# himhan34/Intensity_based_LiDAR_SLAM_for_me-

Measured on NVIDIA B200. Metric: scan-to-map registrations/sec (OS0-64 frame, 100k-pt map), higher is better.
Workload: dtype f32 k-NN / f64 fit+solve

## Files before the change

### include/ilsm.h

```cpp
#ifndef ILSM_H_
#define ILSM_H_

#include <stddef.h>
#include <stdint.h>

#ifdef __cplusplus
extern "C" {
#endif

#define ILSM_ABI_VERSION 1

#if defined(__GNUC__)
#define ILSM_API __attribute__((visibility("default")))
#else
#define ILSM_API
#endif

typedef enum ilsm_status {
  ILSM_OK = 0,
  ILSM_ERR_INVALID_ARG = -1,
  ILSM_ERR_CUDA = -2,
  ILSM_ERR_NO_DEVICE = -3,
  ILSM_ERR_NOT_ENOUGH_MAP = -4,
  ILSM_ERR_OUT_OF_MEMORY = -5,
// ... 6 lines not shown
  ILSM_FAILURE = 2
} ilsm_termination;

typedef struct ilsm_ctx ilsm_ctx;
typedef struct ilsm_map ilsm_map;

ILSM_API int ilsm_abi_version(void);
ILSM_API const char* ilsm_last_error(void);

ILSM_API int ilsm_create(int device, ilsm_ctx** out);
ILSM_API void ilsm_destroy(ilsm_ctx* ctx);
ILSM_API int ilsm_sync(ilsm_ctx* ctx);
ILSM_API int ilsm_set_async(ilsm_ctx* ctx, int on);
ILSM_API void* ilsm_stream(ilsm_ctx* ctx);

ILSM_API int ilsm_host_register(void* ptr, size_t bytes);
ILSM_API int ilsm_host_unregister(void* ptr);

ILSM_API int ilsm_map_create(ilsm_ctx* ctx, ilsm_map** out);
ILSM_API void ilsm_map_destroy(ilsm_map* map);
ILSM_API int ilsm_map_size(const ilsm_map* map);

ILSM_API int ilsm_map_build(ilsm_map* map, const float* xyz, int n, int stride_bytes, float cell);
ILSM_API int ilsm_map_build_dev(ilsm_map* map, const float* d_xyz, int n, int stride_bytes, float cell);
ILSM_API int ilsm_map_build_pair_dev(ilsm_map* map_a, const float* d_xyz_a, int n_a, ilsm_map* map_b, const float* d_xyz_b, int n_b,
                                     int stride_bytes, float cell);
ILSM_API int ilsm_map_join(ilsm_map* map);

#define ILSM_INSERT_APPEND 0
#define ILSM_INSERT_NEAREST_TO_CENTRE 1
ILSM_API int ilsm_map_insert(ilsm_map* map, const float* xyz, int n, int stride_bytes, int policy, float leaf);

ILSM_API int ilsm_map_points(ilsm_map* map, float* out_xyzi, int capacity, int* n_out);

ILSM_API int ilsm_knn(ilsm_map* map, const float* q_xyz, int nq, int stride_bytes, int k, float max_dist, int32_t* idx,
             float* d2);
ILSM_API int ilsm_knn_dev(ilsm_map* map, const float* d_q_xyz, int nq, int stride_bytes, int k, float max_dist,
                 int32_t* d_idx, float* d_d2);

typedef struct ilsm_reg_opts {
  int32_t outer_iterations;
  int32_t max_num_iterations;
  double huber_a;
  float knn_gate_sq;
  float reserved0;
  double line_eig_ratio;
  double plane_tol;
  int32_t min_corner_map;
  int32_t min_surf_map;
} ilsm_reg_opts;

ILSM_API void ilsm_reg_opts_default(ilsm_reg_opts* o);

typedef struct ilsm_solve_summary {
  int32_t termination;
  int32_t iterations;
  int32_t num_successful_steps;
  int32_t num_unsuccessful_steps;
  int32_t num_edge_factors;
  int32_t num_plane_factors;
  int32_t num_evaluations;
  int32_t reserved;
  double initial_cost;
  double final_cost;
} ilsm_solve_summary;

// ... 285 lines not shown
```

### intensity_based_lidar_slam_for_me-_b200/binding.py

```python
from __future__ import annotations

import ctypes as C
import os

import numpy as np

from . import _build

ILSM_OK = 0
ILSM_ERR_NOT_ENOUGH_MAP = -4
CONVERGENCE, NO_CONVERGENCE, FAILURE = 0, 1, 2
MAX_OUTER = 8


class IlsmError(RuntimeError):
    def __init__(self, code, msg):
        super().__init__(f"ilsm error {code}: {msg}")
        self.code = code


class RegOpts(C.Structure):
    _fields_ = [("outer_iterations", C.c_int32), ("max_num_iterations", C.c_int32), ("huber_a", C.c_double),
                ("knn_gate_sq", C.c_float), ("reserved0", C.c_float), ("line_eig_ratio", C.c_double),
                ("plane_tol", C.c_double), ("min_corner_map", C.c_int32), ("min_surf_map", C.c_int32)]
# ... 64 lines not shown

def pc2_layout_ouster() -> Pc2Layout:
    lay = Pc2Layout()
    load_library().ilsm_pc2_layout_ouster(C.byref(lay))
    return lay


def load_library(path: str | None = None):
    global _lib
    if _lib is not None:
        return _lib
    path = path or _build.LIB
    if not os.path.exists(path):
        raise IlsmError(-100, f"{path} not built; run `python -c 'import __graft_entry__ as g; g.build()'`")
    lib = C.CDLL(path)
    vp, i32, f32, f64 = C.c_void_p, C.c_int, C.c_float, C.c_double
    sig = {
        "ilsm_abi_version": (i32, []),
        "ilsm_last_error": (C.c_char_p, []),
        "ilsm_create": (i32, [i32, C.POINTER(vp)]),
        "ilsm_destroy": (None, [vp]),
        "ilsm_sync": (i32, [vp]),
        "ilsm_stream": (vp, [vp]),
        "ilsm_set_async": (i32, [vp, i32]),
        "ilsm_map_create": (i32, [vp, C.POINTER(vp)]),
        "ilsm_map_destroy": (None, [vp]),
        "ilsm_map_size": (i32, [vp]),
        "ilsm_map_build": (i32, [vp, vp, i32, i32, f32]),
        "ilsm_map_build_dev": (i32, [vp, vp, i32, i32, f32]),
        "ilsm_map_join": (i32, [vp]),
        "ilsm_knn": (i32, [vp, vp, i32, i32, i32, f32, vp, vp]),
        "ilsm_map_insert": (i32, [vp, vp, i32, i32, i32, f32]),
        "ilsm_map_points": (i32, [vp, vp, i32, C.POINTER(i32)]),
        "ilsm_knn_dev": (i32, [vp, vp, i32, i32, i32, f32, vp, vp]),
        "ilsm_reg_opts_default": (None, [C.POINTER(RegOpts)]),
        "ilsm_register": (i32, [vp, vp, vp, vp, i32, vp, i32, i32, vp, vp, C.POINTER(RegOpts), C.POINTER(RegReport)]),
        "ilsm_register_dev": (i32, [vp, vp, vp, vp, i32, vp, i32, i32, vp, C.POINTER(RegOpts), vp]),
        "ilsm_associate": (i32, [vp, vp, vp, vp, i32, vp, i32, i32, vp, vp, C.POINTER(RegOpts), vp, vp, vp]),
        "ilsm_project": (i32, [vp, vp, i32, i32, i32, vp, vp, vp]),
        "ilsm_project_dev": (i32, [vp, vp, i32, i32, i32, vp, vp, vp]),
        "ilsm_extract_features": (i32, [vp, vp, i32, i32, f32, C.POINTER(Features)]),
        "ilsm_voxelgrid": (i32, [vp, vp, i32, i32, f32, vp, C.POINTER(i32)]),
        "ilsm_map_build_pair_dev": (i32, [vp, vp, i32, vp, vp, i32, i32, C.c_float]),
        "ilsm_register_frame": (i32, [vp, vp, vp, vp, i32, i32, C.c_float, C.c_float, C.c_float, vp, vp, vp, vp, vp]),
        "ilsm_register_frame_dev": (i32, [vp, vp, vp, vp, i32, i32, C.c_float, C.c_float, C.c_float, vp, vp]),
        "ilsm_sc_create": (i32, [vp, C.POINTER(vp)]),
        "ilsm_sc_destroy": (None, [vp]),
        "ilsm_sc_size": (i32, [vp]),
        "ilsm_sc_make": (i32, [vp, vp, i32, i32, vp]),
        "ilsm_sc_add": (i32, [vp, vp, i32]),
        "ilsm_sc_add_dev": (i32, [vp, vp, i32]),
        "ilsm_sc_query_topk": (i32, [vp, vp, i32, i32, i32, vp, vp, vp]),
        "ilsm_sc_query_topk_dev": (i32, [vp, vp, i32, i32, i32, vp, vp, vp]),
        "ilsm_sc_merge_topk_dev": (i32, [vp, vp, i32, i32, vp]),
        "ilsm_sc_merge_topk": (i32, [vp, vp, vp, i32, i32, vp, vp, vp]),
        "ilsm_sc_query_candidates": (i32, [vp, vp, i32, i32, vp, vp, vp, vp]),
        "ilsm_sc_query_topk_batch": (i32, [vp, vp, i32, i32, i32, i32, vp, vp, vp]),
        "ilsm_sc_query_topk_batch_dev": (i32, [vp, vp, i32, i32, i32, i32, vp]),
        "ilsm_sc_prefilter_debug": (i32, [vp, vp, i32, i32, vp, vp]),
        "ilsm_sc_nccl_unique_id": (i32, [vp]),
        "ilsm_sc_init_nccl_rank": (i32, [vp, vp, i32, i32]),
        "ilsm_sc_init_nccl": (i32, [vp, vp, i32, i32]),
        "ilsm_sc_nccl_version": (i32, [vp]),
        "ilsm_sc_query_topk_sharded": (i32, [vp, vp, i32, i32, i32, i32, vp, vp, vp]),
        "ilsm_sc_query_topk_sharded_dev": (i32, [vp, vp, i32, i32, i32, i32, vp]),
        "ilsm_odometry": (i32, [vp, vp, vp, vp, i32, vp, i32, i32, vp, vp, C.POINTER(RegOpts), C.POINTER(RegReport), vp]),
# ... 300 lines not shown
        return int(self._lib.ilsm_map_size(self._h))

    def set_input_cloud(self, cloud, cell: float = 0.0):
        a, n, stride = _cloud(cloud)
        _check(self._lib.ilsm_map_build(self._h, _ptr(a), n, stride, cell))
        return self

    build = set_input_cloud

    def build_dev(self, d_ptr: int, n: int, stride: int, cell: float = 0.0):
        _check(self._lib.ilsm_map_build_dev(self._h, d_ptr, n, stride, cell))
        return self

    def build_pair_dev(self, d_ptr: int, n: int, other: "LocalMap", d_ptr_other: int, n_other: int, stride: int, cell: float = 0.0):
        _check(self._lib.ilsm_map_build_pair_dev(self._h, d_ptr, n, other._h, d_ptr_other, n_other, stride, cell))
        return self

    def join(self):
        _check(self._lib.ilsm_map_join(self._h))
        return self

    def add_points(self, cloud, downsample=True, downsample_size=0.4):
        a, n, stride = _cloud(cloud)
        _check(self._lib.ilsm_map_insert(self._h, _ptr(a), n, stride, 1 if downsample else 0, downsample_size))
        return self

    def points(self):
        n = C.c_int(0)
        _check(self._lib.ilsm_map_points(self._h, None, 0, C.byref(n)))
        out = np.empty((max(n.value, 1), 4), np.float32)
        _check(self._lib.ilsm_map_points(self._h, _ptr(out), n.value, C.byref(n)))
        return out[:n.value]

    def nearest_k_search(self, queries, k: int = 5, max_dist: float = 0.0):
        q, nq, stride = _cloud(queries)
        idx = np.empty((nq, k), np.int32)
        d2 = np.empty((nq, k), np.float32)
        _check(self._lib.ilsm_knn(self._h, _ptr(q), nq, stride, k, max_dist, _ptr(idx), _ptr(d2)))
        return idx, d2

    def knn_dev(self, d_q_ptr: int, nq: int, stride: int, k: int, max_dist: float, d_idx_ptr: int, d_d2_ptr: int):
        _check(self._lib.ilsm_knn_dev(self._h, d_q_ptr, nq, stride, k, max_dist, d_idx_ptr, d_d2_ptr))


def merge_topk(dist, ids, shifts, k):
    d = np.ascontiguousarray(dist, np.float64).ravel()
    i = np.ascontiguousarray(ids, np.int32).ravel()
    s = np.ascontiguousarray(shifts, np.int32).ravel()
    od, oi, os_ = np.zeros(k), np.zeros(k, np.int32), np.zeros(k, np.int32)
    _check(load_library().ilsm_sc_merge_topk(_ptr(d), _ptr(i), _ptr(s), len(d), k, _ptr(od), _ptr(oi), _ptr(os_)))
    return od, oi, os_


class ScanContextDb:
    NUM_EXCLUDE_RECENT = 50
    SC_DIST_THRES = 0.13

    def __init__(self, ctx: Context):
        self._ctx = ctx
        self._lib = ctx._lib
        h = C.c_void_p()
        _check(self._lib.ilsm_sc_create(ctx._h, C.byref(h)))
        self._h = h

    def close(self):
        if getattr(self, "_h", None) and getattr(self._ctx, "_h", None):
# ... 334 lines not shown
```

### intensity_based_lidar_slam_for_me-_b200/csrc/api.cu

```cuda
#include <stdio.h>
#include <string.h>

#include <atomic>
#include <new>

#include "ilsm_host.hpp"

namespace ilsm {

static thread_local char g_err[512] = "";

int fail(int code, const char* msg) {
  snprintf(g_err, sizeof(g_err), "%s", msg);
  return code;
}
int fail_cuda(cudaError_t e, const char* where) {
  snprintf(g_err, sizeof(g_err), "CUDA error %d (%s) at %s", (int)e, cudaGetErrorString(e), where);
  cudaGetLastError();
  return ILSM_ERR_CUDA;
}
static std::atomic<long long> g_launches{0};
void count_launches(int k) { g_launches.fetch_add(k, std::memory_order_relaxed); }

int check_launch(const char* where) {
  cudaError_t e = cudaGetLastError();
  if (e != cudaSuccess) return fail_cuda(e, where);
  return ILSM_OK;
}

int eval_only_launch(Ctx* c, double* d_out, const double* d_pose7 = nullptr, double huber_a = 0.0);
int factors_export(Ctx* c, ilsm_factor* d_out);
int sc_merge_dev(Ctx* ctx, const void* d_packed, int shards, int k, void* d_out, int batch = 1, size_t shard_stride = 0);
void sc_nccl_release(ScDb& d);

struct Pose7 {
  double v[7];
};
// ... 20 lines not shown
    else if (t < 7) pose7[t] = st->xt[t - 4];
    if (report) {
      const int words = (int)(sizeof(ilsm_reg_report) / 4);
      const int32_t* src = reinterpret_cast<const int32_t*>(&st->report);
      int32_t* dst = reinterpret_cast<int32_t*>(report);
      for (int w = t; w < words; w += blockDim.x) dst[w] = src[w];
    }
  }
}

int Ctx::init(int dev) {
  int count = 0;
  cudaError_t e = cudaGetDeviceCount(&count);
  if (e != cudaSuccess || count <= 0) {
    cudaGetLastError();
    return fail(ILSM_ERR_NO_DEVICE, "no CUDA device available (libilsm_cuda has no CPU fallback)");
  }
  if (dev < 0 || dev >= count) return fail(ILSM_ERR_INVALID_ARG, "ilsm_create: device index out of range");
  device = dev;
  ILSM_CUDA(cudaSetDevice(dev));
  cudaDeviceProp prop;
  ILSM_CUDA(cudaGetDeviceProperties(&prop, dev));
  sm_count = prop.multiProcessorCount;
  ILSM_CUDA(cudaStreamCreateWithFlags(&stream, cudaStreamNonBlocking));
  ILSM_CUDA(cudaStreamCreateWithFlags(&aux, cudaStreamNonBlocking));
  ILSM_CUDA(cudaEventCreateWithFlags(&ev_fork, cudaEventDisableTiming));
  ILSM_CUDA(cudaEventCreateWithFlags(&ev_join, cudaEventDisableTiming));
  int rc;
  if ((rc = lm.reserve(1))) return rc;
  ILSM_CUDA(cudaMemsetAsync(lm.p, 0, sizeof(LmState), stream));
  if ((rc = pinned.reserve(4096))) return rc;
  ILSM_CUDA(cudaStreamSynchronize(stream));
  if (const char* e2 = getenv("ILSM_KNN_BINNED_MIN")) knn_binned_min = atoi(e2) > 0 ? atoi(e2) : 0x7fffffff;
  if (const char* e3 = getenv("ILSM_KNN_GROUP")) {
    const int gsz = atoi(e3);
    if (gsz == 1 || gsz == 2 || gsz == 4 || gsz == 8 || gsz == 16 || gsz == 32) knn_group = gsz;
  }
  return ILSM_OK;
}

void Ctx::release() {
  if (fe_graph_exec) cudaGraphExecDestroy(fe_graph_exec), fe_graph_exec = nullptr;
  if (stream) cudaStreamSynchronize(stream);
  fe.vg_hash.release(), fe.vg_keys.release(), fe.vg_state.release(), fe.vg_chunk.release(), fe.chunk_hist.release(), fe.chunk_base.release(), fe.scanid.release(), fe.picked.release(), fe.ori.release(), fe.curv.release(), fe.stats.release();
  fe.src_index.release(), fe.label.release(), fe.sort_ind.release(), fe.ring_sharp.release(), fe.ring_lsharp.release();
  fe.ring_flat.release(), fe.sharp.release(), fe.lsharp.release(), fe.flat.release(), fe.counts.release();
  fe.cloud.release(), fe.ring_pts.release(), fe.ring_out.release(), fe.lflat.release(), fe.vox_packed.release();
  fe.pc2.release(), fe.raw.release(), fe.img.release(), fe.track.release(), fe.vox_out.release(), fe.vox_n.release();
  lm.release(), partials.release(), stack_raw.release(), out_idx.release(), out_d2.release(), pinned.release();
  rf_lsharp.release(), rf_stack_c.release(), rf_stack_s.release(), rf_stack_n.release();
  if (qbin) qbin->release(), delete qbin, qbin = nullptr;
  qwork.release();
  fac.type.release(), fac.p.release(), fac.a.release(), fac.b.release(), fac.knn_idx.release(), fac.knn_d2.release();
  if (aux) cudaStreamSynchronize(aux), cudaStreamDestroy(aux);
  if (ev_fork) cudaEventDestroy(ev_fork);
  if (ev_join) cudaEventDestroy(ev_join);
  if (stream) cudaStreamDestroy(stream);
  stream = nullptr, aux = nullptr, ev_fork = nullptr, ev_join = nullptr;
}

void Map::release() {
  if (stream) cudaStreamSynchronize(stream);
  if (ready) cudaEventDestroy(ready);
  if (ctx_done) cudaEventDestroy(ctx_done);
  if (stream) cudaStreamDestroy(stream);
  stream = nullptr, ready = nullptr, ctx_done = nullptr;
// ... 164 lines not shown

ILSM_API int ilsm_map_insert(ilsm_map* map, const float* xyz, int n, int stride_bytes, int policy, float leaf) {
  if (!map || (n > 0 && !xyz)) return fail(ILSM_ERR_INVALID_ARG, "ilsm_map_insert: null argument");
  if (n < 0 || !valid_stride(stride_bytes)) return fail(ILSM_ERR_INVALID_ARG, "ilsm_map_insert: bad n/stride");
  Map& m = map->m;
  std::lock_guard<std::mutex> lk(m.ctx->mu);
  ILSM_CUDA(cudaSetDevice(m.ctx->device));
  if (m.table_size == 0) {
    int rc0 = m.build_dev(nullptr, 0, 16, m.cell);
    if (rc0) return rc0;
  }
  size_t bytes = (size_t)n * stride_bytes;
  int rc;
  if ((rc = m.raw.reserve(bytes / 4 + 4))) return rc;
  ILSM_CUDA(cudaEventRecord(m.ctx_done, m.ctx->stream));
  ILSM_CUDA(cudaStreamWaitEvent(m.stream, m.ctx_done, 0));
  if (bytes) ILSM_CUDA(cudaMemcpyAsync(m.raw.p, xyz, bytes, cudaMemcpyHostToDevice, m.stream));
  if ((rc = m.insert_dev(m.raw.p, n, stride_bytes, policy, leaf))) return rc;
  ILSM_CUDA(cudaStreamSynchronize(m.stream));
  return ILSM_OK;
}

ILSM_API int ilsm_map_points(ilsm_map* map, float* out_xyzi, int capacity, int* n_out) {
  if (!map || !n_out || (capacity > 0 && !out_xyzi)) return fail(ILSM_ERR_INVALID_ARG, "ilsm_map_points: null argument");
  Map& m = map->m;
  std::lock_guard<std::mutex> lk(m.ctx->mu);
  ILSM_CUDA(cudaSetDevice(m.ctx->device));
  *n_out = m.n;
  const int k = m.n < capacity ? m.n : capacity;
  if (k > 0) {
    ILSM_CUDA(cudaStreamSynchronize(m.stream));
    ILSM_CUDA(cudaMemcpy(out_xyzi, m.orig.p, (size_t)k * 16, cudaMemcpyDeviceToHost));
  }
  return ILSM_OK;
}

ILSM_API int ilsm_knn_dev(ilsm_map* map, const float* d_q, int nq, int stride_bytes, int k, float max_dist, int32_t* d_idx,
                 float* d_d2) {
  if (!map || (nq > 0 && (!d_q || !d_idx || !d_d2))) return fail(ILSM_ERR_INVALID_ARG, "ilsm_knn_dev: null argument");
  std::lock_guard<std::mutex> lk(map->m.ctx->mu);
  ILSM_CUDA(cudaSetDevice(map->m.ctx->device));
  return map->m.knn_dev(d_q, nq, stride_bytes, k, max_dist, d_idx, d_d2);
}

ILSM_API int ilsm_knn(ilsm_map* map, const float* q, int nq, int stride_bytes, int k, float max_dist, int32_t* idx, float* d2) {
  if (!map || (nq > 0 && (!q || !idx || !d2))) return fail(ILSM_ERR_INVALID_ARG, "ilsm_knn: null argument");
  if (nq < 0 || !valid_stride(stride_bytes) || k < 1 || k > 8) return fail(ILSM_ERR_INVALID_ARG, "ilsm_knn: bad nq/k/stride");
  Map& m = map->m;
  Ctx& c = *m.ctx;
  std::lock_guard<std::mutex> lk(c.mu);
  ILSM_CUDA(cudaSetDevice(c.device));
  if (nq == 0) return ILSM_OK;
  size_t bytes = (size_t)nq * stride_bytes;
  int rc;
  if ((rc = c.stack_raw.reserve(bytes / 4 + 4)) || (rc = c.out_idx.reserve((size_t)nq * k)) ||
      (rc = c.out_d2.reserve((size_t)nq * k)))
    return rc;
  ILSM_CUDA(cudaMemcpyAsync(c.stack_raw.p, q, bytes, cudaMemcpyHostToDevice, c.stream));
  if ((rc = m.knn_dev(c.stack_raw.p, nq, stride_bytes, k, max_dist, c.out_idx.p, c.out_d2.p))) return rc;
  ILSM_CUDA(cudaMemcpyAsync(idx, c.out_idx.p, (size_t)nq * k * 4, cudaMemcpyDeviceToHost, c.stream));
  ILSM_CUDA(cudaMemcpyAsync(d2, c.out_d2.p, (size_t)nq * k * 4, cudaMemcpyDeviceToHost, c.stream));
  ILSM_CUDA(cudaStreamSynchronize(c.stream));
  return ILSM_OK;
}

static int check_reg_args(ilsm_ctx* ctx, ilsm_map* mc, ilsm_map* ms, const float* corner, int nc, const float* surf,
// ... 675 lines not shown
```

### intensity_based_lidar_slam_for_me-_b200/csrc/ilsm_host.hpp

```cpp
#pragma once
#include <cuda_runtime.h>
#include <limits.h>
#include <stddef.h>
#include <stdint.h>
#include <string.h>

#include <mutex>
#include <string>

#include "../../include/ilsm.h"
#include "ilsm_internal.cuh"

namespace ilsm {

int fail(int code, const char* msg);
int fail_cuda(cudaError_t e, const char* where);
int check_launch(const char* where);
void count_launches(int k);

#define ILSM_CUDA(call)                                        \
  do {                                                         \
    cudaError_t e__ = (call);                                  \
    if (e__ != cudaSuccess) return ::ilsm::fail_cuda(e__, #call); \
  } while (0)
// ... 158 lines not shown
  DevBuf<int> stats, src_index, label, sort_ind, ring_sharp, ring_lsharp, ring_flat, sharp, lsharp, flat, counts;
  DevBuf<u64> vg_keys;
  DevBuf<VgState> vg_state;
  DevBuf<int> vg_chunk;
  DevBuf<uint32_t> vg_hash;
  DevBuf<int> chunk_hist, chunk_base;
  DevBuf<float4> cloud, ring_pts, ring_out, lflat, vox_packed;
  DevBuf<float> raw;
  DevBuf<unsigned char> pc2;
  DevBuf<unsigned char> img;
  DevBuf<float4> track;
  DevBuf<float4> vox_out;
  DevBuf<int> vox_n;
  int n_in = 0, ring_cap = 0;
};

struct Ctx {
  int device = 0;
  int sm_count = 148;
  cudaStream_t stream = nullptr;
  cudaStream_t aux = nullptr;
  cudaEvent_t ev_fork = nullptr, ev_join = nullptr;
  std::mutex mu;
  DevBuf<LmState> lm;
  DevBuf<double> partials;
  DevBuf<float> stack_raw;
  DevBuf<int32_t> out_idx;
  DevBuf<float> out_d2;
  PinnedBuf<unsigned char> pinned;
  FactorBufs fac;
  FeBufs fe;
  const int* d_stack_counts = nullptr;
  int solve_wide = -1;
  DevBuf<float4> rf_lsharp, rf_stack_c, rf_stack_s;
  DevBuf<int> rf_stack_n;
  Map* qbin = nullptr;
  DevBuf<int> qwork;
  int knn_group = 8;
  int knn_binned_min = 8192;
  size_t partial_blocks = 0;
  bool bulk_attr_set = false;

  int init(int dev);
  void release();
  static constexpr size_t kPinSite = 1024, kPinPoseIn = 2048;
  static_assert(offsetof(LmState, xq) == 0 && offsetof(LmState, xt) == 4 * sizeof(double) && kLmHostBytes <= kPinSite,
                "the LM read-back overlaps the call sites' area");
  int upload_pose(const double q[4], const double t[3], cudaStream_t s) {
    double* p = reinterpret_cast<double*>(pinned.p + kPinPoseIn);
    for (int i = 0; i < 4; ++i) p[i] = q[i];
    for (int i = 0; i < 3; ++i) p[4 + i] = t[i];
    ILSM_CUDA(cudaMemcpyAsync(lm.p->xq, p, 7 * sizeof(double), cudaMemcpyHostToDevice, s));
    return ILSM_OK;
  }
  int read_back_lm(cudaStream_t s) {
    ILSM_CUDA(cudaMemcpyAsync(pinned.p, lm.p, kLmHostBytes, cudaMemcpyDeviceToHost, s));
    return ILSM_OK;
  }
  void lm_result(double q[4], double t[3], ilsm_reg_report* report) const {
    const double* x = reinterpret_cast<const double*>(pinned.p);
    for (int i = 0; i < 4; ++i) q[i] = x[i];
    for (int i = 0; i < 3; ++i) t[i] = x[4 + i];
    if (report) memcpy(report, pinned.p + offsetof(LmState, report), sizeof(*report));
  }
  bool async_build = false;
  int associate_dev(Map* mc, Map* ms, const float* d_corner, int nc, const float* d_surf, int ns, int stride_bytes,
// ... 70 lines not shown
```

### intensity_based_lidar_slam_for_me-_b200/csrc/ilsm_internal.cuh

```cuda
#pragma once
#include <cuda_runtime.h>
#include <stdint.h>

namespace ilsm {

typedef unsigned long long u64;

constexpr u64 kEmptyKey = 0xFFFFFFFFFFFFFFFFull;
constexpr u64 kSentinel = 0xFFFFFFFFFFFFFFFFull;
constexpr int kCoordOff = 1 << 20;
constexpr int kCoordLim = (1 << 20) - 4;
constexpr int kMaxRing = 6;

struct __align__(16) GridCell {
  u64 key;
  uint32_t start;
  uint32_t count;
};

struct GridView {
  const GridCell* cells;
  const float4* sorted;
  const float4* orig;
  const int* bbox;
  uint32_t mask;
  int log2_size;
  float cell, inv_cell;
  int n;
};

__device__ __forceinline__ void pdl_entry() {
  asm volatile("griddepcontrol.wait;" ::: "memory");
  asm volatile("griddepcontrol.launch_dependents;" ::: "memory");
}

__device__ __forceinline__ int voxel_coord(float x, float inv_cell) { return __float2int_rd(__fmul_rn(x, inv_cell)); }

__device__ __forceinline__ u64 pack_voxel(int cx, int cy, int cz) {
  return ((u64)(uint32_t)(cx + kCoordOff) << 42) | ((u64)(uint32_t)(cy + kCoordOff) << 21) |
         (u64)(uint32_t)(cz + kCoordOff);
}

__device__ __forceinline__ uint32_t hash_voxel(u64 key, int log2_size) {
  return (uint32_t)((key * 0x9E3779B97F4A7C15ull) >> (64 - log2_size));
}

__device__ __forceinline__ float dist2_rn(float qx, float qy, float qz, float px, float py, float pz) {
  float dx = __fsub_rn(qx, px), dy = __fsub_rn(qy, py), dz = __fsub_rn(qz, pz);
  return __fadd_rn(__fadd_rn(__fmul_rn(dx, dx), __fmul_rn(dy, dy)), __fmul_rn(dz, dz));
}

__device__ __forceinline__ u64 pack_cand(float d2, uint32_t idx) { return ((u64)__float_as_uint(d2) << 32) | idx; }
__device__ __forceinline__ float cand_d2(u64 k) { return __uint_as_float((uint32_t)(k >> 32)); }
__device__ __forceinline__ int cand_idx(u64 k) { return (int)(uint32_t)(k & 0xFFFFFFFFull); }

__device__ __forceinline__ uint4 ldg_cell(const GridCell* c) { return __ldg(reinterpret_cast<const uint4*>(c)); }

__device__ __forceinline__ uint32_t probe_voxel(const GridView& g, u64 key, uint32_t& start) {
  uint32_t slot = hash_voxel(key, g.log2_size);
#pragma unroll 1
  for (;;) {
    uint4 e = ldg_cell(g.cells + slot);
    u64 k = ((u64)e.y << 32) | e.x;
    if (k == key) {
      start = e.z;
      return e.w;
// ... 206 lines not shown
```

### intensity_based_lidar_slam_for_me-_b200/csrc/map_grid.cu

```cuda
#include "ilsm_host.hpp"

namespace ilsm {

struct BuildJob {
  const float* src;
  int n, stride_f, ioff;
  float inv_cell;
  GridCell* cells;
  uint32_t mask;
  int log2_size;
  float4* orig;
  float4* sorted;
  uint32_t *slot_of, *rank_of;
  uint32_t* counters;
  uint32_t* occ;
  int* bbox;
  GridCell* o_cells;
  const uint32_t* o_occ;
  uint32_t* o_counters;
  int* o_bbox;
  int o_cover;
  int blocks;
};
struct BuildJobs {
  BuildJob j[2];
  int nb0;
};

__global__ void grid_clear_kernel(GridCell* cells, uint32_t size, int* bbox, uint32_t* counters) {
  pdl_entry();
  uint32_t i = blockIdx.x * blockDim.x + threadIdx.x;
  if (i < size) {
    uint4 e;
    e.x = 0xFFFFFFFFu, e.y = 0xFFFFFFFFu, e.z = 0u, e.w = 0u;
    reinterpret_cast<uint4*>(cells)[i] = e;
  }
  if (i < 3) bbox[i] = INT_MAX;
  if (i >= 3 && i < 6) bbox[i] = INT_MIN;
  if (i < 8) counters[i] = 0;
}

__device__ __forceinline__ bool load_point(const float* src, int stride_f, int i, float& x, float& y, float& z) {
  const float* p = src + (size_t)i * stride_f;
  x = __ldg(p), y = __ldg(p + 1), z = __ldg(p + 2);
  return isfinite(x) && isfinite(y) && isfinite(z);
}

__global__ void __launch_bounds__(256) grid_count_kernel(BuildJobs jobs) {
  pdl_entry();
  __shared__ uint32_t s_wnew[8];
  __shared__ uint32_t s_obase;
  const int w = (int)blockIdx.x >= jobs.nb0;
  const BuildJob& jb = jobs.j[w];
  const int i = ((int)blockIdx.x - (w ? jobs.nb0 : 0)) * blockDim.x + threadIdx.x;
  const int lane = threadIdx.x & 31;
  const bool in = i < jb.n;
  float x = 0.f, y = 0.f, z = 0.f;
  bool ok = in && load_point(jb.src, jb.stride_f, i, x, y, z);
  if (in) jb.orig[i] = make_float4(x, y, z, jb.ioff >= 0 ? __ldg(jb.src + (size_t)i * jb.stride_f + jb.ioff) : 0.f);
  int cx = 0, cy = 0, cz = 0;
  if (ok) {
    float ux = __fmul_rn(x, jb.inv_cell), uy = __fmul_rn(y, jb.inv_cell), uz = __fmul_rn(z, jb.inv_cell);
    ok = fabsf(ux) < (float)kCoordLim && fabsf(uy) < (float)kCoordLim && fabsf(uz) < (float)kCoordLim;
    cx = __float2int_rd(ux), cy = __float2int_rd(uy), cz = __float2int_rd(uz);
  }
  if (in && !ok) {
    jb.slot_of[i] = 0xFFFFFFFFu;
    atomicAdd(&jb.counters[2], 1u);
  }
  const u64 key = ok ? pack_voxel(cx, cy, cz) : (kEmptyKey - 1ull - (u64)lane);
  const unsigned peers = __match_any_sync(0xffffffffu, key);
  bool created = false;
  uint32_t my_slot = 0;
  if (ok) {
    const int leader = __ffs(peers) - 1;
    uint32_t slot = 0, base = 0;
    if (lane == leader) {
      slot = hash_voxel(key, jb.log2_size);
      for (;;) {
        u64 prev = atomicCAS(&jb.cells[slot].key, kEmptyKey, key);
        if (prev == kEmptyKey) created = true;
        if (prev == kEmptyKey || prev == key) break;
        slot = (slot + 1) & jb.mask;
      }
      base = atomicAdd(&jb.cells[slot].count, (uint32_t)__popc(peers));
      my_slot = slot;
    }
    slot = __shfl_sync(peers, slot, leader);
    base = __shfl_sync(peers, base, leader);
    jb.slot_of[i] = slot;
    jb.rank_of[i] = base + (uint32_t)__popc(peers & ((1u << lane) - 1u));
  }
  const unsigned newb = __ballot_sync(0xffffffffu, created);
  const int warp = threadIdx.x >> 5;
  if (lane == 0) s_wnew[warp] = (uint32_t)__popc(newb);
  __syncthreads();
  if (threadIdx.x == 0) {
    uint32_t tot = 0;
#pragma unroll
    for (int k = 0; k < 8; ++k) tot += s_wnew[k];
    s_obase = tot ? atomicAdd(&jb.counters[4], tot) : 0u;
  }
  __syncthreads();
  if (created) {
    uint32_t wb = 0;
#pragma unroll
    for (int k = 0; k < 8; ++k)
      if (k < warp) wb += s_wnew[k];
    jb.occ[s_obase + wb + (uint32_t)__popc(newb & ((1u << lane) - 1u))] = my_slot;
  }
}

__global__ void __launch_bounds__(256) grid_alloc_kernel(BuildJobs jobs) {
  pdl_entry();
  const int w = (int)blockIdx.x >= jobs.nb0;
  const BuildJob& jb = jobs.j[w];
  const uint32_t li = ((uint32_t)blockIdx.x - (w ? (uint32_t)jobs.nb0 : 0u)) * blockDim.x + threadIdx.x;
  const uint32_t size = jb.counters[4];
  uint32_t cnt = 0;
  int lo[3] = {INT_MAX, INT_MAX, INT_MAX}, hi[3] = {INT_MIN, INT_MIN, INT_MIN};
  const uint32_t i = li < size ? jb.occ[li] : 0u;
  if (li < size) {
    uint4 e = *reinterpret_cast<const uint4*>(jb.cells + i);
    cnt = e.w;
    if (cnt) {
      u64 key = ((u64)e.y << 32) | e.x;
      int c[3] = {(int)((key >> 42) & 0x1FFFFF) - kCoordOff, (int)((key >> 21) & 0x1FFFFF) - kCoordOff,
                  (int)(key & 0x1FFFFF) - kCoordOff};
#pragma unroll
      for (int a = 0; a < 3; ++a) lo[a] = hi[a] = c[a];
    }
  }
  __shared__ uint32_t s_wsum[8];
  __shared__ uint32_t s_base;
  const uint32_t lane = threadIdx.x & 31, warp = threadIdx.x >> 5;
  uint32_t inc = cnt;
#pragma unroll
  for (int off = 1; off < 32; off <<= 1) {
    uint32_t v = __shfl_up_sync(0xffffffffu, inc, off);
    if (lane >= (uint32_t)off) inc += v;
  }
  const uint32_t total = __shfl_sync(0xffffffffu, inc, 31);
  if (lane == 31) s_wsum[warp] = inc;
  __syncthreads();
  uint32_t wbase = 0, btotal = 0;
#pragma unroll
  for (int k = 0; k < 8; ++k) {
    if (k < (int)warp) wbase += s_wsum[k];
    btotal += s_wsum[k];
  }
  if (threadIdx.x == 0) s_base = btotal ? atomicAdd(&jb.counters[0], btotal) : 0u;
  __syncthreads();
  if (li < size && cnt) jb.cells[i].start = s_base + wbase + inc - cnt;
#pragma unroll
  for (int a = 0; a < 3; ++a) {
#pragma unroll
    for (int off = 16; off > 0; off >>= 1) {
      lo[a] = min(lo[a], __shfl_xor_sync(0xffffffffu, lo[a], off));
      hi[a] = max(hi[a], __shfl_xor_sync(0xffffffffu, hi[a], off));
    }
  }
  __shared__ int s_lo[3], s_hi[3];
  if (threadIdx.x < 3) s_lo[threadIdx.x] = INT_MAX, s_hi[threadIdx.x] = INT_MIN;
  __syncthreads();
  if (lane == 0 && total) {
#pragma unroll
    for (int a = 0; a < 3; ++a) atomicMin(&s_lo[a], lo[a]), atomicMax(&s_hi[a], hi[a]);
  }
  __syncthreads();
  if (threadIdx.x < 3 && s_lo[threadIdx.x] != INT_MAX) {
    atomicMin(&jb.bbox[threadIdx.x], s_lo[threadIdx.x]);
    atomicMax(&jb.bbox[3 + threadIdx.x], s_hi[threadIdx.x]);
  }
}

__global__ void __launch_bounds__(256) grid_scatter_kernel(BuildJobs jobs) {
  pdl_entry();
  __shared__ int s_last;
  const int w = (int)blockIdx.x >= jobs.nb0;
  const BuildJob& jb = jobs.j[w];
  const int i = ((int)blockIdx.x - (w ? jobs.nb0 : 0)) * blockDim.x + threadIdx.x;
  if (i < jb.n) {
    const uint32_t slot = jb.slot_of[i];
    if (slot != 0xFFFFFFFFu) {
      float4 p = jb.orig[i];
      p.w = __uint_as_float((uint32_t)i);
      jb.sorted[jb.cells[slot].start + jb.rank_of[i]] = p;
    }
  }
  if (jb.o_cover > 0) {
    const uint32_t n_old = jb.o_counters[4];
    for (uint32_t k = (uint32_t)i; k < n_old; k += (uint32_t)jb.blocks * blockDim.x) {
      uint4 e;
      e.x = 0xFFFFFFFFu, e.y = 0xFFFFFFFFu, e.z = 0u, e.w = 0u;
      reinterpret_cast<uint4*>(jb.o_cells)[jb.o_occ[k]] = e;
    }
    __syncthreads();
    if (threadIdx.x == 0) {
      __threadfence();
      s_last = atomicAdd(&jb.counters[6], 1u) == (uint32_t)jb.blocks - 1u;
    }
    __syncthreads();
    if (s_last) {
      if (threadIdx.x < 8) jb.o_counters[threadIdx.x] = 0;
      if (threadIdx.x < 3) jb.o_bbox[threadIdx.x] = INT_MAX;
      if (threadIdx.x >= 3 && threadIdx.x < 6) jb.o_bbox[threadIdx.x] = INT_MIN;
      if (threadIdx.x == 0) jb.counters[6] = 0;
    }
  }
}

template <int K>
__global__ void __launch_bounds__(128) knn_kernel(GridView g, const float* __restrict__ q, int nq, int stride_f, int k_out,
                                                  float max_d2, int32_t* __restrict__ idx, float* __restrict__ d2) {
  pdl_entry();
  __shared__ WarpScratch scratch[4];
  const unsigned lane = threadIdx.x & 31, warp = threadIdx.x >> 5;
  int bb[6];
  load_bbox(g, bb);
  const int nwarps = gridDim.x * 4;
  for (int gid = blockIdx.x * 4 + warp; gid < nq; gid += nwarps) {
    const float* qp = q + (size_t)gid * stride_f;
    const float qx = __ldg(qp), qy = __ldg(qp + 1), qz = __ldg(qp + 2);
    KnnResult<K, false> res;
    knn_search<K, false>(g, bb, qx, qy, qz, max_d2, lane, scratch[warp], res);
    if (lane == 0) {
#pragma unroll
      for (int k = 0; k < K; ++k) {
        if (k < k_out) {
          bool have = res.key[k] != kSentinel;
          idx[(size_t)gid * k_out + k] = have ? cand_idx(res.key[k]) : -1;
          d2[(size_t)gid * k_out + k] = have ? cand_d2(res.key[k]) : __int_as_float(0x7f800000);
        }
      }
    }
  }
}

int knn_binned_dev(Ctx* ctx, Map* m, const float* d_q, int nq, int stride_bytes, int k, float max_dist, int32_t* d_idx, float* d_d2);

static inline int ilog2_ceil(uint32_t v) {
  int l = 0;
// ... 64 lines not shown
  jb.counters = counters.p + 8 * t, jb.occ = occ.p + (size_t)t * occ_cap, jb.bbox = bbox.p + 8 * t;
  jb.o_cells = cells.p + (size_t)o * table_cap, jb.o_occ = occ.p + (size_t)o * occ_cap;
  jb.o_counters = counters.p + 8 * o, jb.o_bbox = bbox.p + 8 * o;
  jb.o_cover = filled_n[o];
  jb.blocks = n_pts > 0 ? (n_pts + 255) / 256 : 0;
  if (n_pts > 0 && filled_n[o] != 0) {
    filled_n[o] = 0;
  } else if (filled_n[o] != 0) {
    jb.o_cover = 0;
  }
  filled_n[t] = n_pts > 0 ? (n_pts > 8 ? n_pts : 8) : 0;
  gen += 1;
  return ILSM_OK;
}

int Map::reserve_points(int n_pts) {
  if (n_pts <= 0) return ILSM_OK;
  int want_log2 = ilog2_ceil(2u * (uint32_t)n_pts);
  if (want_log2 < 10) want_log2 = 10;
  const uint32_t want_size = 1u << want_log2;
  const uint32_t new_cap = want_size > table_cap ? want_size : table_cap;
  const size_t new_occ_cap = (size_t)n_pts + 1 > occ_cap ? (size_t)n_pts + (size_t)n_pts / 2 + 64 : occ_cap;
  if (new_cap == table_cap && new_occ_cap == occ_cap && sorted.cap >= (size_t)n_pts + 1) return ILSM_OK;
  int rc;
  if ((rc = cells.reserve((size_t)2 * new_cap)) || (rc = sorted.reserve(n_pts + 1)) || (rc = orig.reserve(n_pts + 1)) ||
      (rc = slot_of.reserve(n_pts + 1)) || (rc = rank_of.reserve(n_pts + 1)) || (rc = bbox.reserve(16)) ||
      (rc = counters.reserve(16)) || (rc = occ.reserve(2 * new_occ_cap)))
    return rc;
  table_cap = new_cap, occ_cap = new_occ_cap;
  clean_size[0] = clean_size[1] = 0, filled_n[0] = filled_n[1] = 0;
  return ILSM_OK;
}

static int launch_build(BuildJobs& jobs, int n_jobs, cudaStream_t s) {
  const int b0 = jobs.j[0].blocks, b1 = n_jobs > 1 ? jobs.j[1].blocks : 0;
  jobs.nb0 = n_jobs > 1 ? b0 : 0x7fffffff;
  if (b0 + b1 == 0) return ILSM_OK;
  if (n_jobs > 1 && b0 == 0) {
    jobs.j[0] = jobs.j[1];
    jobs.nb0 = 0x7fffffff;
  }
  ILSM_CUDA(launch_pdl(grid_count_kernel, dim3(b0 + b1), dim3(256), 0, s, jobs));
  ILSM_CUDA(launch_pdl(grid_alloc_kernel, dim3(b0 + b1), dim3(256), 0, s, jobs));
  ILSM_CUDA(launch_pdl(grid_scatter_kernel, dim3(b0 + b1), dim3(256), 0, s, jobs));
  count_launches(3);
  return ILSM_OK;
}

int Map::build_dev(const float* d_src, int n_pts, int stride_bytes, float cell_size) {
  if (in_line) {
    cudaStream_t cs = ctx->stream;
    if (pending) ILSM_CUDA(cudaStreamWaitEvent(cs, ready, 0));
    pending = false;
    BuildJobs jobs = {};
    int rc = prepare_build(d_src, n_pts, stride_bytes, cell_size, cs, &jobs.j[0]);
    if (rc) return rc;
    if ((rc = launch_build(jobs, 1, cs))) return rc;
    return check_launch("map_build");
  }
  cudaStream_t s = stream;
  ILSM_CUDA(cudaEventRecord(ctx_done, ctx->stream));
  ILSM_CUDA(cudaStreamWaitEvent(s, ctx_done, 0));
  if (pending) ILSM_CUDA(cudaStreamWaitEvent(s, ready, 0));
  BuildJobs jobs = {};
  int rc = prepare_build(d_src, n_pts, stride_bytes, cell_size, s, &jobs.j[0]);
  if (rc) return rc;
  if ((rc = launch_build(jobs, 1, s))) return rc;
  ILSM_CUDA(cudaEventRecord(ready, s));
  pending = true;
  return check_launch("map_build");
}

int build_pair_dev(Map* a, const float* d_a, int na, Map* b, const float* d_b, int nb, int stride_bytes, float cell_size) {
  if (!a || !b || a == b || a->ctx != b->ctx) return fail(ILSM_ERR_INVALID_ARG, "map_build_pair: two maps of one context expected");
  Ctx* ctx = a->ctx;
  const bool in_line = a->in_line && b->in_line;
  cudaStream_t s = in_line ? ctx->stream : a->stream;
  if (in_line) {
    if (a->pending) ILSM_CUDA(cudaStreamWaitEvent(s, a->ready, 0));
    if (b->pending) ILSM_CUDA(cudaStreamWaitEvent(s, b->ready, 0));
    a->pending = b->pending = false;
  } else {
    ILSM_CUDA(cudaEventRecord(a->ctx_done, ctx->stream));
    ILSM_CUDA(cudaStreamWaitEvent(s, a->ctx_done, 0));
    if (a->pending) ILSM_CUDA(cudaStreamWaitEvent(s, a->ready, 0));
    if (b->pending) ILSM_CUDA(cudaStreamWaitEvent(s, b->ready, 0));
  }
  BuildJobs jobs = {};
  int rc;
  if ((rc = a->prepare_build(d_a, na, stride_bytes, cell_size, s, &jobs.j[0])) || (rc = b->prepare_build(d_b, nb, stride_bytes, cell_size, s, &jobs.j[1])))
    return rc;
  if ((rc = launch_build(jobs, 2, s))) return rc;
  if (!in_line) {
    ILSM_CUDA(cudaEventRecord(a->ready, s));
    ILSM_CUDA(cudaEventRecord(b->ready, s));
    a->pending = b->pending = true;
  }
  return check_launch("map_build_pair");
}

GridView Map::view() const {
  GridView g;
  g.cells = cells.p + (size_t)cur * table_cap;
  g.sorted = sorted.p;
  g.orig = orig.p;
  g.bbox = bbox.p + 8 * cur;
  g.mask = table_size - 1;
  g.log2_size = log2_size;
  g.cell = cell;
  g.inv_cell = inv_cell;
  g.n = n;
  return g;
}

template <int K>
static int launch_knn(const GridView& g, const float* d_q, int nq, int stride_f, int k, float max_d2, int32_t* d_idx,
                       float* d_d2, cudaStream_t s, int sm_count) {
  long long blocks = ((long long)nq + 3) / 4, cap = (long long)sm_count * 4 * 4;
  if (blocks > cap) blocks = cap;
  ILSM_CUDA(launch_pdl(knn_kernel<K>, dim3((unsigned)blocks), dim3(128), 0, s, g, d_q, nq, stride_f, k, max_d2, d_idx, d_d2));
  return ILSM_OK;
}

int Map::knn_dev(const float* d_q, int nq, int stride_bytes, int k, float max_dist, int32_t* d_idx, float* d_d2) {
  if (nq < 0 || k < 1 || k > 8 || (stride_bytes % 4) != 0 || stride_bytes < 12)
// ... 26 lines not shown
```

### intensity_based_lidar_slam_for_me-_b200/csrc/registration.cu

```cuda
#include "ilsm_host.hpp"

namespace ilsm {

__device__ __forceinline__ void jacobi_rot(double& app, double& aqq, double& apq, double& arp, double& arq, double& v0p,
                                           double& v0q, double& v1p, double& v1q, double& v2p, double& v2q) {
  if (apq == 0.0) return;
  const double h = aqq - app;
  const double t = (h >= 0.0 ? 2.0 : -2.0) * apq * frcp(fabs(h) + fsqrt(h * h + 4.0 * apq * apq));
  const double c = frsqrt(t * t + 1.0), s = t * c;
  app -= t * apq;
  aqq += t * apq;
  apq = 0.0;
  double x = arp, y = arq;
  arp = c * x - s * y;
  arq = s * x + c * y;
  x = v0p, y = v0q, v0p = c * x - s * y, v0q = s * x + c * y;
  x = v1p, y = v1q, v1p = c * x - s * y, v1q = s * x + c * y;
  x = v2p, y = v2q, v2p = c * x - s * y, v2q = s * x + c * y;
}

__device__ __forceinline__ bool fit_line(const float (&nb)[5][3], double ratio, double (&pa)[3], double (&pb)[3]) {
  double cx = 0, cy = 0, cz = 0;
#pragma unroll
  for (int j = 0; j < 5; ++j) cx = cx + (double)nb[j][0], cy = cy + (double)nb[j][1], cz = cz + (double)nb[j][2];
// ... 826 lines not shown
}
__device__ __forceinline__ void cluster_sync_all() {
  asm volatile("barrier.cluster.arrive.release.aligned;\n\tbarrier.cluster.wait.acquire.aligned;" ::: "memory");
}
__device__ __forceinline__ void dsmem_push_f64(uint32_t remote_addr, double v, uint32_t remote_mbar) {
  asm volatile("st.async.shared::cluster.mbarrier::complete_tx::bytes.b64 [%0], %1, [%2];" ::"r"(remote_addr),
               "l"(__double_as_longlong(v)), "r"(remote_mbar)
               : "memory");
}
__device__ __forceinline__ void mbar_wait_cluster(uint32_t bar, uint32_t parity) {
  asm volatile(
      "{\n"
      ".reg .pred p;\n"
      "XWAIT_LOOP:\n"
      "mbarrier.try_wait.parity.acquire.cluster.shared::cta.b64 p, [%0], %1;\n"
      "@p bra XWAIT_DONE;\n"
      "bra XWAIT_LOOP;\n"
      "XWAIT_DONE:\n"
      "}\n" ::"r"(bar),
      "r"(parity)
      : "memory");
}

struct SolveParams {
  int max_iter, pass, arm;
  double huber_a;
  double* d_pose7_out;
  ilsm_reg_report* d_report_out;
};

template <int kCS, int kThr>
__global__ void __cluster_dims__(kCS, 1, 1) __launch_bounds__(kThr, 1)
    solve_cluster_kernel(FactorView fv, int n, LmState* st, SolveParams prm, const int* __restrict__ d_counts) {
  pdl_entry();
  __shared__ double core[kCoreWords];
  if (d_counts) n = d_counts[0] + d_counts[1];
  __shared__ double red[kThr / 32][kSumStride];
  __shared__ double recv[2][kCS][kSumStride];
  __shared__ __align__(8) unsigned long long xbar[2];
  __shared__ double tot[kSumStride];
  constexpr uint32_t kXferBytes = kCS * kSumStride * 8;
  const uint32_t rank = cluster_ctarank();
  const int tid = threadIdx.x, lane = tid & 31, warp = tid >> 5;
  const int cl_tid = tid * kCS + (int)rank, cl_n = kCS * kThr;
  LmState* s = reinterpret_cast<LmState*>(core);

  int type0 = 0;
  float4 p0 = make_float4(0.f, 0.f, 0.f, 0.f);
  double4 a0 = make_double4(0, 0, 0, 0), b0 = a0;
  if (cl_tid < n) {
    type0 = fv.type[cl_tid];
    if (type0) {
      p0 = fv.p[cl_tid];
      a0 = fv.a[cl_tid];
      if (type0 == 1) b0 = fv.b[cl_tid];
    }
  }
  {
    const double* src = reinterpret_cast<const double*>(st);
    for (int w = tid; w < kCoreWords; w += kThr) core[w] = src[w];
  }
  if (tid == 0) {
    mbar_init(smem_u32(&xbar[0]), 1), mbar_init(smem_u32(&xbar[1]), 1);
    asm volatile("fence.mbarrier_init.release.cluster;" ::: "memory");
    mbar_expect_tx(smem_u32(&xbar[0]), kXferBytes), mbar_expect_tx(smem_u32(&xbar[1]), kXferBytes);
  }
  __syncthreads();
  if (tid == 0 && prm.arm) lm_arm(s, prm.max_iter, prm.huber_a, prm.pass);
  cluster_sync_all();
  ilsm_reg_report* rep = rank == 0 ? &st->report : nullptr;

#ifdef ILSM_DEBUG_TIMING
#define STAMP(k) do { if (rank == 0 && tid == 0 && e < 6) st->dbg[e * 8 + (k)] = clock64(); } while (0)
#else
#define STAMP(k) do { } while (0)
#endif
#pragma unroll 1
  for (int e = 0; s->status == 0; ++e) {
    STAMP(0);
    const double q[4] = {s->cq[0], s->cq[1], s->cq[2], s->cq[3]};
    const double t[3] = {s->ct[0], s->ct[1], s->ct[2]};
    const double huber_a = s->huber_a;
    double acc[kSumStride];
#pragma unroll
    for (int i = 0; i < kSumStride; ++i) acc[i] = 0.0;
#pragma unroll 1
    for (int i = cl_tid, it = 0; i < n; i += cl_n, ++it) {
      int ty = type0;
      float4 pf = p0;
      double4 fa = a0, fb = b0;
      if (it > 0) {
        ty = fv.type[i];
        if (ty) pf = fv.p[i], fa = fv.a[i], fb = fv.b[i];
      }
      if (ty) eval_factor(ty, pf, fa, fb, q, t, huber_a, acc);
    }
    STAMP(1);
    const double mine = warp_reduce_transpose(acc, lane);
    red[warp][lane] = mine;
    __syncthreads();
    STAMP(2);
    const int buf = e & 1;
// ... 433 lines not shown
```

Measured before the change: 13470.

## Fuse grid count/alloc/scatter into one cooperative kernel; overlap solve prologue via PDL

The three map-build kernels (count, alloc, scatter) become device functions. When the grid fits in one resident wave, they run inside a single cooperative launch, separated by spin-wait barriers built on an atomic job counter. This removes two kernel launches and their dependency gaps per build, but relies on all blocks being co-resident and on the counter being reset correctly. The solve cluster kernel now does its mbarrier setup and cluster sync before griddepcontrol.wait, so that setup overlaps the previous kernel's tail. The change also adds an ilsm_map_grid export for reading back the hash grid, plus an env override to force the three-launch path.

```diff
diff --git a/include/ilsm.h b/include/ilsm.h
--- a/include/ilsm.h
+++ b/include/ilsm.h
@@ -62,6 +62,9 @@
 ILSM_API int ilsm_map_insert(ilsm_map* map, const float* xyz, int n, int stride_bytes, int policy, float leaf);
 
 ILSM_API int ilsm_map_points(ilsm_map* map, float* out_xyzi, int capacity, int* n_out);
+
+ILSM_API int ilsm_map_grid(ilsm_map* map, uint64_t* keys, uint32_t* starts, uint32_t* counts, int capacity, int* n_cells,
+                           float* sorted_xyzi, int32_t bbox[6]);
 
 ILSM_API int ilsm_knn(ilsm_map* map, const float* q_xyz, int nq, int stride_bytes, int k, float max_dist, int32_t* idx,
              float* d2);
diff --git a/intensity_based_lidar_slam_for_me-_b200/binding.py b/intensity_based_lidar_slam_for_me-_b200/binding.py
--- a/intensity_based_lidar_slam_for_me-_b200/binding.py
+++ b/intensity_based_lidar_slam_for_me-_b200/binding.py
@@ -120,6 +120,7 @@
         "ilsm_knn": (i32, [vp, vp, i32, i32, i32, f32, vp, vp]),
         "ilsm_map_insert": (i32, [vp, vp, i32, i32, i32, f32]),
         "ilsm_map_points": (i32, [vp, vp, i32, C.POINTER(i32)]),
+        "ilsm_map_grid": (i32, [vp, vp, vp, vp, i32, C.POINTER(i32), vp, vp]),
         "ilsm_knn_dev": (i32, [vp, vp, i32, i32, i32, f32, vp, vp]),
         "ilsm_reg_opts_default": (None, [C.POINTER(RegOpts)]),
         "ilsm_register": (i32, [vp, vp, vp, vp, i32, vp, i32, i32, vp, vp, C.POINTER(RegOpts), C.POINTER(RegReport)]),
@@ -486,6 +487,14 @@
         _check(self._lib.ilsm_map_points(self._h, _ptr(out), n.value, C.byref(n)))
         return out[:n.value]
 
+    def grid(self):
+        n = C.c_int(0)
+        _check(self._lib.ilsm_map_grid(self._h, None, None, None, 0, C.byref(n), None, None))
+        keys, starts, counts = np.empty(n.value, np.uint64), np.empty(n.value, np.uint32), np.empty(n.value, np.uint32)
+        pts, bbox = np.empty((max(len(self), 1), 4), np.float32), np.empty(6, np.int32)
+        _check(self._lib.ilsm_map_grid(self._h, _ptr(keys), _ptr(starts), _ptr(counts), n.value, C.byref(n), _ptr(pts), _ptr(bbox)))
+        return keys, starts, counts, pts[:len(self)], bbox
+
     def nearest_k_search(self, queries, k: int = 5, max_dist: float = 0.0):
         q, nq, stride = _cloud(queries)
         idx = np.empty((nq, k), np.int32)
diff --git a/intensity_based_lidar_slam_for_me-_b200/csrc/api.cu b/intensity_based_lidar_slam_for_me-_b200/csrc/api.cu
--- a/intensity_based_lidar_slam_for_me-_b200/csrc/api.cu
+++ b/intensity_based_lidar_slam_for_me-_b200/csrc/api.cu
@@ -3,6 +3,7 @@
 
 #include <atomic>
 #include <new>
+#include <vector>
 
 #include "ilsm_host.hpp"
 
@@ -89,6 +90,8 @@
   if ((rc = pinned.reserve(4096))) return rc;
   ILSM_CUDA(cudaStreamSynchronize(stream));
   if (const char* e2 = getenv("ILSM_KNN_BINNED_MIN")) knn_binned_min = atoi(e2) > 0 ? atoi(e2) : 0x7fffffff;
+  if (const char* e4 = getenv("ILSM_BUILD_LAUNCHES"))
+    if (atoi(e4) == 3) build_coop_blocks = 0;
   if (const char* e3 = getenv("ILSM_KNN_GROUP")) {
     const int gsz = atoi(e3);
     if (gsz == 1 || gsz == 2 || gsz == 4 || gsz == 8 || gsz == 16 || gsz == 32) knn_group = gsz;
@@ -319,6 +322,30 @@
     ILSM_CUDA(cudaStreamSynchronize(m.stream));
     ILSM_CUDA(cudaMemcpy(out_xyzi, m.orig.p, (size_t)k * 16, cudaMemcpyDeviceToHost));
   }
+  return ILSM_OK;
+}
+
+ILSM_API int ilsm_map_grid(ilsm_map* map, uint64_t* keys, uint32_t* starts, uint32_t* counts, int capacity, int* n_cells,
+                           float* sorted_xyzi, int32_t bbox[6]) {
+  if (!map || !n_cells || (capacity > 0 && (!keys || !starts || !counts))) return fail(ILSM_ERR_INVALID_ARG, "ilsm_map_grid: null argument");
+  Map& m = map->m;
+  std::lock_guard<std::mutex> lk(m.ctx->mu);
+  ILSM_CUDA(cudaSetDevice(m.ctx->device));
+  *n_cells = 0;
+  if (m.table_size == 0) return ILSM_OK;
+  ILSM_CUDA(cudaStreamSynchronize(m.stream));
+  ILSM_CUDA(cudaStreamSynchronize(m.ctx->stream));
+  std::vector<GridCell> tab(m.table_size);
+  ILSM_CUDA(cudaMemcpy(tab.data(), m.cur_cells(), tab.size() * sizeof(GridCell), cudaMemcpyDeviceToHost));
+  int k = 0;
+  for (const GridCell& c : tab) {
+    if (c.key == kEmptyKey) continue;
+    if (k < capacity) keys[k] = c.key, starts[k] = c.start, counts[k] = c.count;
+    ++k;
+  }
+  *n_cells = k;
+  if (sorted_xyzi && m.n > 0) ILSM_CUDA(cudaMemcpy(sorted_xyzi, m.sorted.p, (size_t)m.n * 16, cudaMemcpyDeviceToHost));
+  if (bbox) ILSM_CUDA(cudaMemcpy(bbox, m.view().bbox, 6 * sizeof(int32_t), cudaMemcpyDeviceToHost));
   return ILSM_OK;
 }
 
diff --git a/intensity_based_lidar_slam_for_me-_b200/csrc/ilsm_host.hpp b/intensity_based_lidar_slam_for_me-_b200/csrc/ilsm_host.hpp
--- a/intensity_based_lidar_slam_for_me-_b200/csrc/ilsm_host.hpp
+++ b/intensity_based_lidar_slam_for_me-_b200/csrc/ilsm_host.hpp
@@ -214,6 +214,7 @@
   FeBufs fe;
   const int* d_stack_counts = nullptr;
   int solve_wide = -1;
+  int build_coop_blocks = -1;
   DevBuf<float4> rf_lsharp, rf_stack_c, rf_stack_s;
   DevBuf<int> rf_stack_n;
   Map* qbin = nullptr;
diff --git a/intensity_based_lidar_slam_for_me-_b200/csrc/ilsm_internal.cuh b/intensity_based_lidar_slam_for_me-_b200/csrc/ilsm_internal.cuh
--- a/intensity_based_lidar_slam_for_me-_b200/csrc/ilsm_internal.cuh
+++ b/intensity_based_lidar_slam_for_me-_b200/csrc/ilsm_internal.cuh
@@ -29,9 +29,11 @@
   int n;
 };
 
+__device__ __forceinline__ void pdl_wait() { asm volatile("griddepcontrol.wait;" ::: "memory"); }
+__device__ __forceinline__ void pdl_launch_dependents() { asm volatile("griddepcontrol.launch_dependents;" ::: "memory"); }
 __device__ __forceinline__ void pdl_entry() {
-  asm volatile("griddepcontrol.wait;" ::: "memory");
-  asm volatile("griddepcontrol.launch_dependents;" ::: "memory");
+  pdl_wait();
+  pdl_launch_dependents();
 }
 
 __device__ __forceinline__ int voxel_coord(float x, float inv_cell) { return __float2int_rd(__fmul_rn(x, inv_cell)); }
diff --git a/intensity_based_lidar_slam_for_me-_b200/csrc/map_grid.cu b/intensity_based_lidar_slam_for_me-_b200/csrc/map_grid.cu
--- a/intensity_based_lidar_slam_for_me-_b200/csrc/map_grid.cu
+++ b/intensity_based_lidar_slam_for_me-_b200/csrc/map_grid.cu
@@ -46,8 +46,7 @@
   return isfinite(x) && isfinite(y) && isfinite(z);
 }
 
-__global__ void __launch_bounds__(256) grid_count_kernel(BuildJobs jobs) {
-  pdl_entry();
+__device__ __forceinline__ void grid_count(const BuildJobs& jobs) {
   __shared__ uint32_t s_wnew[8];
   __shared__ uint32_t s_obase;
   const int w = (int)blockIdx.x >= jobs.nb0;
@@ -111,8 +110,7 @@
   }
 }
 
-__global__ void __launch_bounds__(256) grid_alloc_kernel(BuildJobs jobs) {
-  pdl_entry();
+__device__ __forceinline__ void grid_alloc(const BuildJobs& jobs) {
   const int w = (int)blockIdx.x >= jobs.nb0;
   const BuildJob& jb = jobs.j[w];
   const uint32_t li = ((uint32_t)blockIdx.x - (w ? (uint32_t)jobs.nb0 : 0u)) * blockDim.x + threadIdx.x;
@@ -174,8 +172,7 @@
   }
 }
 
-__global__ void __launch_bounds__(256) grid_scatter_kernel(BuildJobs jobs) {
-  pdl_entry();
+__device__ __forceinline__ void grid_scatter(const BuildJobs& jobs) {
   __shared__ int s_last;
   const int w = (int)blockIdx.x >= jobs.nb0;
   const BuildJob& jb = jobs.j[w];
@@ -208,6 +205,42 @@
       if (threadIdx.x == 0) jb.counters[6] = 0;
     }
   }
+}
+
+__global__ void __launch_bounds__(256) grid_count_kernel(BuildJobs jobs) {
+  pdl_entry();
+  grid_count(jobs);
+}
+__global__ void __launch_bounds__(256) grid_alloc_kernel(BuildJobs jobs) {
+  pdl_entry();
+  grid_alloc(jobs);
+}
+__global__ void __launch_bounds__(256) grid_scatter_kernel(BuildJobs jobs) {
+  pdl_entry();
+  grid_scatter(jobs);
+}
+
+__device__ __forceinline__ void job_barrier(const BuildJob& jb, uint32_t k) {
+  __syncthreads();
+  if (threadIdx.x == 0) {
+    volatile uint32_t* arrived = jb.counters + 1;
+    const uint32_t target = k * (uint32_t)jb.blocks;
+    __threadfence();
+    atomicAdd(jb.counters + 1, 1u);
+    while (*arrived < target) __nanosleep(20);
+    __threadfence();
+  }
+  __syncthreads();
+}
+
+__global__ void __launch_bounds__(256) grid_build_kernel(BuildJobs jobs) {
+  pdl_entry();
+  const BuildJob& jb = jobs.j[(int)blockIdx.x >= jobs.nb0];
+  grid_count(jobs);
+  job_barrier(jb, 1);
+  grid_alloc(jobs);
+  job_barrier(jb, 2);
+  grid_scatter(jobs);
 }
 
 template <int K>
@@ -338,13 +371,31 @@
   return ILSM_OK;
 }
 
-static int launch_build(BuildJobs& jobs, int n_jobs, cudaStream_t s) {
+static int launch_build(Ctx* ctx, BuildJobs& jobs, int n_jobs, cudaStream_t s) {
   const int b0 = jobs.j[0].blocks, b1 = n_jobs > 1 ? jobs.j[1].blocks : 0;
   jobs.nb0 = n_jobs > 1 ? b0 : 0x7fffffff;
   if (b0 + b1 == 0) return ILSM_OK;
   if (n_jobs > 1 && b0 == 0) {
     jobs.j[0] = jobs.j[1];
     jobs.nb0 = 0x7fffffff;
+  }
+  if (ctx->build_coop_blocks < 0) {
+    int per_sm = 0;
+    ILSM_CUDA(cudaOccupancyMaxActiveBlocksPerMultiprocessor(&per_sm, grid_build_kernel, 256, 0));
+    ctx->build_coop_blocks = per_sm * ctx->sm_count;
+  }
+  if (b0 + b1 <= ctx->build_coop_blocks) {
+    cudaLaunchConfig_t cfg = {};
+    cfg.gridDim = dim3(b0 + b1), cfg.blockDim = dim3(256), cfg.dynamicSmemBytes = 0, cfg.stream = s;
+    cudaLaunchAttribute attr[2];
+    attr[0].id = cudaLaunchAttributeCooperative;
+    attr[0].val.cooperative = 1;
+    attr[1].id = cudaLaunchAttributeProgrammaticStreamSerialization;
+    attr[1].val.programmaticStreamSerializationAllowed = 1;
+    cfg.attrs = attr, cfg.numAttrs = 2;
+    ILSM_CUDA(cudaLaunchKernelEx(&cfg, grid_build_kernel, jobs));
+    count_launches(1);
+    return ILSM_OK;
   }
   ILSM_CUDA(launch_pdl(grid_count_kernel, dim3(b0 + b1), dim3(256), 0, s, jobs));
   ILSM_CUDA(launch_pdl(grid_alloc_kernel, dim3(b0 + b1), dim3(256), 0, s, jobs));
@@ -361,7 +412,7 @@
     BuildJobs jobs = {};
     int rc = prepare_build(d_src, n_pts, stride_bytes, cell_size, cs, &jobs.j[0]);
     if (rc) return rc;
-    if ((rc = launch_build(jobs, 1, cs))) return rc;
+    if ((rc = launch_build(ctx, jobs, 1, cs))) return rc;
     return check_launch("map_build");
   }
   cudaStream_t s = stream;
@@ -371,7 +422,7 @@
   BuildJobs jobs = {};
   int rc = prepare_build(d_src, n_pts, stride_bytes, cell_size, s, &jobs.j[0]);
   if (rc) return rc;
-  if ((rc = launch_build(jobs, 1, s))) return rc;
+  if ((rc = launch_build(ctx, jobs, 1, s))) return rc;
   ILSM_CUDA(cudaEventRecord(ready, s));
   pending = true;
   return check_launch("map_build");
@@ -396,7 +447,7 @@
   int rc;
   if ((rc = a->prepare_build(d_a, na, stride_bytes, cell_size, s, &jobs.j[0])) || (rc = b->prepare_build(d_b, nb, stride_bytes, cell_size, s, &jobs.j[1])))
     return rc;
-  if ((rc = launch_build(jobs, 2, s))) return rc;
+  if ((rc = launch_build(ctx, jobs, 2, s))) return rc;
   if (!in_line) {
     ILSM_CUDA(cudaEventRecord(a->ready, s));
     ILSM_CUDA(cudaEventRecord(b->ready, s));
diff --git a/intensity_based_lidar_slam_for_me-_b200/csrc/registration.cu b/intensity_based_lidar_slam_for_me-_b200/csrc/registration.cu
--- a/intensity_based_lidar_slam_for_me-_b200/csrc/registration.cu
+++ b/intensity_based_lidar_slam_for_me-_b200/csrc/registration.cu
@@ -882,9 +882,8 @@
 template <int kCS, int kThr>
 __global__ void __cluster_dims__(kCS, 1, 1) __launch_bounds__(kThr, 1)
     solve_cluster_kernel(FactorView fv, int n, LmState* st, SolveParams prm, const int* __restrict__ d_counts) {
-  pdl_entry();
+  pdl_launch_dependents();
   __shared__ double core[kCoreWords];
-  if (d_counts) n = d_counts[0] + d_counts[1];
   __shared__ double red[kThr / 32][kSumStride];
   __shared__ double recv[2][kCS][kSumStride];
   __shared__ __align__(8) unsigned long long xbar[2];
@@ -895,6 +894,14 @@
   const int cl_tid = tid * kCS + (int)rank, cl_n = kCS * kThr;
   LmState* s = reinterpret_cast<LmState*>(core);
 
+  if (tid == 0) {
+    mbar_init(smem_u32(&xbar[0]), 1), mbar_init(smem_u32(&xbar[1]), 1);
+    asm volatile("fence.mbarrier_init.release.cluster;" ::: "memory");
+    mbar_expect_tx(smem_u32(&xbar[0]), kXferBytes), mbar_expect_tx(smem_u32(&xbar[1]), kXferBytes);
+  }
+  cluster_sync_all();
+  pdl_wait();
+  if (d_counts) n = d_counts[0] + d_counts[1];
   int type0 = 0;
   float4 p0 = make_float4(0.f, 0.f, 0.f, 0.f);
   double4 a0 = make_double4(0, 0, 0, 0), b0 = a0;
@@ -910,14 +917,9 @@
     const double* src = reinterpret_cast<const double*>(st);
     for (int w = tid; w < kCoreWords; w += kThr) core[w] = src[w];
   }
-  if (tid == 0) {
-    mbar_init(smem_u32(&xbar[0]), 1), mbar_init(smem_u32(&xbar[1]), 1);
-    asm volatile("fence.mbarrier_init.release.cluster;" ::: "memory");
-    mbar_expect_tx(smem_u32(&xbar[0]), kXferBytes), mbar_expect_tx(smem_u32(&xbar[1]), kXferBytes);
-  }
   __syncthreads();
   if (tid == 0 && prm.arm) lm_arm(s, prm.max_iter, prm.huber_a, prm.pass);
-  cluster_sync_all();
+  __syncthreads();
   ilsm_reg_report* rep = rank == 0 ? &st->report : nullptr;
 
 #ifdef ILSM_DEBUG_TIMING
```

After: 13730, median of 6. +1.9%, better.
